# david-strejc/fei

Measured on AMD Instinct MI355X. Metric: agent tok/s (llama3-8b local decode, 1 agent/GPU), higher is better.
Workload: dtype bf16; 1 GPU; model=llama3-8b, global_batch=1, seq_len=512, parallelism=dp1 (1 agent per GPU, weak scaling), hip_graph=True, stream_engine=False

## Files before the change

fei_amd/models/llama.py:

```python

from __future__ import annotations

import math
import os
from dataclasses import dataclass
from typing import Dict, List, Optional

import torch
import torch.nn.functional as F

from fei_amd import ops
from fei_amd.engine.config import ModelSpec
from fei_amd.ops import reference as ref
from fei_amd.parallel.pg import ParallelContext, all_gather_cat, all_reduce_sum


@dataclass
class LayerWeights:
    norm_attn: torch.Tensor
    wqkv: torch.Tensor
    wo: torch.Tensor
    norm_mlp: torch.Tensor
    wgu: torch.Tensor
    wdown: torch.Tensor
# ... 7 lines not shown
        dtype: torch.dtype = torch.bfloat16,
        tp: Optional[ParallelContext] = None,
        seed: int = 1234,
        max_seq_len: Optional[int] = None,
    ):
        self.spec = spec
        self.device = device
        self.dtype = dtype
        self.tp = tp or ParallelContext()
        self.max_seq_len = max_seq_len or spec.max_seq_len
        tp_size = self.tp.world_size if self.tp.is_distributed else 1
        if spec.num_kv_heads % tp_size or spec.num_heads % tp_size or \
                spec.intermediate_size % tp_size or spec.vocab_size % tp_size:
            raise ValueError(f"model {spec.name} not divisible by tp={tp_size}")
        self.tp_size = tp_size
        self.tp_rank = self.tp.rank if self.tp.is_distributed else 0
        self.hq_l = spec.num_heads // tp_size
        self.hkv_l = spec.num_kv_heads // tp_size
        self.inter_l = spec.intermediate_size // tp_size
        self.vocab_l = spec.vocab_size // tp_size
        self.D = spec.head_dim
        self._init_weights(seed)
        self.rope = ref.rope_table(self.max_seq_len, self.D, spec.rope_theta,
                                   device=device)
        self.prefetch_mb = int(os.environ.get("FEI_PREFETCH", "0") or 0)
        self._pf_stream = None
        self._pf_sink = None
        self.norm_precomp = os.environ.get("FEI_NORM_PRECOMP", "0") == "1"


    def _rand(self, gen, *shape, scale: float) -> torch.Tensor:
        w = torch.randn(*shape, generator=gen, device=self.device,
                        dtype=torch.float32) * scale
        return w.to(self.dtype)

    def _init_weights(self, seed: int) -> None:
        s = self.spec
        gen = torch.Generator(device=self.device)
        gen.manual_seed(seed)
        C = s.hidden_size
        sc = 1.0 / math.sqrt(C)
        self.emb = self._rand(gen, s.vocab_size, C, scale=0.02)
        self.layers: List[LayerWeights] = []
        r = self.tp_rank
        for _ in range(s.num_layers):
            wq = self._rand(gen, s.num_heads * self.D, C, scale=sc)
            wk = self._rand(gen, s.num_kv_heads * self.D, C, scale=sc)
            wv = self._rand(gen, s.num_kv_heads * self.D, C, scale=sc)
            wo = self._rand(gen, C, s.num_heads * self.D, scale=sc / math.sqrt(2 * s.num_layers))
            wg = self._rand(gen, s.intermediate_size, C, scale=sc)
            wu = self._rand(gen, s.intermediate_size, C, scale=sc)
            wd = self._rand(gen, C, s.intermediate_size,
                            scale=1.0 / math.sqrt(s.intermediate_size) / math.sqrt(2 * s.num_layers))
            wq = wq.view(s.num_heads, self.D, C)[r * self.hq_l:(r + 1) * self.hq_l].reshape(-1, C)
            wk = wk.view(s.num_kv_heads, self.D, C)[r * self.hkv_l:(r + 1) * self.hkv_l].reshape(-1, C)
            wv = wv.view(s.num_kv_heads, self.D, C)[r * self.hkv_l:(r + 1) * self.hkv_l].reshape(-1, C)
            wo = wo.view(C, s.num_heads, self.D)[:, r * self.hq_l:(r + 1) * self.hq_l].reshape(C, -1)
            wg = wg[r * self.inter_l:(r + 1) * self.inter_l]
            wu = wu[r * self.inter_l:(r + 1) * self.inter_l]
            wd = wd[:, r * self.inter_l:(r + 1) * self.inter_l]
            self.layers.append(LayerWeights(
                norm_attn=torch.ones(C, device=self.device, dtype=self.dtype),
                wqkv=torch.cat([wq, wk, wv], dim=0).contiguous(),
                wo=wo.contiguous(),
                norm_mlp=torch.ones(C, device=self.device, dtype=self.dtype),
                wgu=torch.cat([wg, wu], dim=0).contiguous(),
                wdown=wd.contiguous(),
            ))
        self.norm_f = torch.ones(C, device=self.device, dtype=self.dtype)
        lm = self._rand(gen, s.vocab_size, C, scale=sc)
        self.lm_head = lm[r * self.vocab_l:(r + 1) * self.vocab_l].contiguous()
        self.vocab_offset = r * self.vocab_l

    def quantize_fp8(self) -> None:
        self.fp8 = []
        for lw in self.layers:
            self.fp8.append({
                "wqkv": ops.quant_fp8(lw.wqkv),
                "wo": ops.quant_fp8(lw.wo),
                "wgu": ops.quant_fp8(lw.wgu),
                "wdown": ops.quant_fp8(lw.wdown),
            })
        self.fp8_lm_head = ops.quant_fp8(self.lm_head)

    def param_bytes(self) -> int:
        total = self.emb.numel() + self.norm_f.numel() + self.lm_head.numel()
        for lw in self.layers:
            for t in (lw.norm_attn, lw.wqkv, lw.wo, lw.norm_mlp, lw.wgu, lw.wdown):
                total += t.numel()
        return total * self.emb.element_size()


    def new_kv_cache(self, batch: int, max_seq: Optional[int] = None,
                     kv_quant: Optional[str] = None):
        max_seq = max_seq or self.max_seq_len
        shape = (batch, self.hkv_l, max_seq, self.D)
        if kv_quant == "fp8":
            return (
                [ops.QuantKV.zeros(shape, self.device)
                 for _ in range(self.spec.num_layers)],
                [ops.QuantKV.zeros(shape, self.device)
                 for _ in range(self.spec.num_layers)],
            )
        if kv_quant is not None:
            raise ValueError(f"unknown kv_quant {kv_quant!r}")
        return (
            [torch.zeros(shape, device=self.device, dtype=self.dtype)
             for _ in range(self.spec.num_layers)],
            [torch.zeros(shape, device=self.device, dtype=self.dtype)
             for _ in range(self.spec.num_layers)],
        )


    def _qkv_views(self, qkv: torch.Tensor, B: int, S: Optional[int] = None):
        D = self.D
        W = qkv.shape[-1]
        off_k = self.hq_l * D
        off_v = off_k + self.hkv_l * D
        if S is None:
            q = qkv.as_strided((B, self.hq_l, D), (W, D, 1))
            k = qkv.as_strided((B, self.hkv_l, D), (W, D, 1), storage_offset=qkv.storage_offset() + off_k)
            v = qkv.as_strided((B, self.hkv_l, D), (W, D, 1), storage_offset=qkv.storage_offset() + off_v)
        else:
            q = qkv.as_strided((B, S, self.hq_l, D), (S * W, W, D, 1))
            k = qkv.as_strided((B, S, self.hkv_l, D), (S * W, W, D, 1), storage_offset=qkv.storage_offset() + off_k)
            v = qkv.as_strided((B, S, self.hkv_l, D), (S * W, W, D, 1), storage_offset=qkv.storage_offset() + off_v)
        return q, k, v


    def forward_decode(
        self,
        token: torch.Tensor,
        pos: torch.Tensor,
        k_caches: List[torch.Tensor],
        v_caches: List[torch.Tensor],
        attn_splits: int = 32,
        workspace=None,
        fused_attn: bool = False,
        attn_out: Optional[torch.Tensor] = None,
        fused_norm: bool = False,
        gather_logits: bool = True,
    ) -> torch.Tensor:
        if fused_norm and self.tp_size == 1 and token.shape[0] == 1 and \
                self.spec.hidden_size * 2 <= 32 * 1024:
            return self._forward_decode_fused_norm(
                token, pos, k_caches, v_caches, attn_splits, workspace,
                fused_attn, attn_out)
        s = self.spec
        B = token.shape[0]
        h = F.embedding(token.long(), self.emb)
        scale = 1.0 / math.sqrt(self.D)
        n_layers = len(self.layers)
        x = ops.rmsnorm(h, self.layers[0].norm_attn, s.norm_eps)
        for li, lw in enumerate(self.layers):
            qkv = ops.linear_decode(x, lw.wqkv)
            q, k, v = self._qkv_views(qkv, B)
            if fused_attn:
                att = ops.attn_decode_fused(q, k, v, k_caches[li],
                                            v_caches[li], pos, self.rope,
                                            scale=scale, out=attn_out)
            else:
                att = ops.attn_decode(q, k_caches[li], v_caches[li], pos,
                                      splits=attn_splits, scale=scale,
                                      workspace=workspace, out=attn_out,
                                      k=k, v=v, table=self.rope, layer=li)
            o = ops.linear_decode(att.reshape(B, -1), lw.wo)
            all_reduce_sum(o, self.tp)
            x, h = ops.fused_add_rmsnorm(o, h, lw.norm_mlp, s.norm_eps)
            act = ops.gemv_swiglu(x, lw.wgu)
            d = ops.linear_decode(act, lw.wdown)
            all_reduce_sum(d, self.tp)
            next_norm = (self.layers[li + 1].norm_attn if li + 1 < n_layers
                         else self.norm_f)
            x, h = ops.fused_add_rmsnorm(d, h, next_norm, s.norm_eps)
        logits = ops.linear_decode(x, self.lm_head)
        if gather_logits:
            logits = all_gather_cat(logits, dim=-1, ctx=self.tp)
        return logits

    def forward_decode_stream(self, token, pos, k_caches, v_caches,
                              ws: dict, bufs) -> torch.Tensor:
        s = self.spec
        h = F.embedding(token.long(), self.emb)
        bufs[0].copy_(h.to(bufs[0].dtype))
        scale = 1.0 / math.sqrt(self.D)
        cur, nxt = bufs
        for li, lw in enumerate(self.layers):
            ops.stream_layer(cur, nxt, lw, s, k_caches[li], v_caches[li],
                             self.rope, pos, ws, li, scale)
            cur, nxt = nxt, cur
        return ops.gemv_norm(cur, self.norm_f, self.lm_head, s.norm_eps)

    def _ssq_slots(self, B: int, device) -> torch.Tensor:
        buf = getattr(self, "_ssq", None)
        if buf is None or buf.shape[1] != B or buf.device != device:
            buf = torch.zeros(2 * len(self.layers), B, dtype=torch.float32,
                              device=device)
            self._ssq = buf
        return buf

    def _forward_decode_fused_norm(self, token, pos, k_caches, v_caches,
                                   attn_splits, workspace, fused_attn,
                                   attn_out):
        s = self.spec
        B = token.shape[0]
        fp8 = getattr(self, "fp8", None)
        if fp8 is not None and (B != 1 or s.hidden_size * 2 > 32 * 1024):
            fp8 = None
        h = F.embedding(token.long(), self.emb).contiguous()
        scale = 1.0 / math.sqrt(self.D)
        ssq = (self._ssq_slots(B, h.device)
               if (self.norm_precomp and fp8 is None and h.is_cuda) else None)
        if ssq is not None:
            ssq.zero_()
        pf = self.prefetch_mb > 0 and fp8 is None and h.is_cuda
        if pf and self._pf_stream is None:
            self._pf_stream = torch.cuda.Stream()
            self._pf_sink = torch.zeros(1, dtype=torch.float32,
                                        device=h.device)
        for li, lw in enumerate(self.layers):
            if fp8 is not None:
                q8 = fp8[li]
                qkv = ops.gemv_norm_fp8(h, lw.norm_attn, *q8["wqkv"],
                                        s.norm_eps)
            else:
                qkv = ops.gemv_norm(
                    h, lw.norm_attn, lw.wqkv, s.norm_eps,
                    ssq=ssq[2 * li - 1] if (ssq is not None and li > 0) else None)
            if pf:
                ev = torch.cuda.Event()
                ev.record()
                with torch.cuda.stream(self._pf_stream):
                    self._pf_stream.wait_event(ev)
                    ops.prefetch(lw.wgu, self.prefetch_mb << 20,
                                 self._pf_sink)
            q, k, v = self._qkv_views(qkv, B)
            if fused_attn:
                att = ops.attn_decode_fused(q, k, v, k_caches[li],
                                            v_caches[li], pos, self.rope,
                                            scale=scale, out=attn_out)
            else:
                att = ops.attn_decode(q, k_caches[li], v_caches[li], pos,
                                      splits=attn_splits, scale=scale,
                                      workspace=workspace, out=attn_out,
                                      k=k, v=v, table=self.rope, layer=li)
            if fp8 is not None:
                ops.gemv_res_fp8(att.reshape(B, -1), *q8["wo"], h)
                act = ops.gemv_swiglu_norm_fp8(h, lw.norm_mlp, *q8["wgu"],
                                               s.norm_eps)
                ops.gemv_res_fp8(act, *q8["wdown"], h)
            else:
                ops.gemv_res(att.reshape(B, -1), lw.wo, h,
                             ssq_out=ssq[2 * li] if ssq is not None else None)
                act = ops.gemv_swiglu_norm(
                    h, lw.norm_mlp, lw.wgu, s.norm_eps,
                    ssq=ssq[2 * li] if ssq is not None else None)
                ops.gemv_res(act, lw.wdown, h,
                             ssq_out=ssq[2 * li + 1] if ssq is not None else None)
        if pf:
            torch.cuda.current_stream().wait_stream(self._pf_stream)
        if fp8 is not None:
            return ops.gemv_norm_fp8(h, self.norm_f, *self.fp8_lm_head,
                                     s.norm_eps)
        return ops.gemv_norm(h, self.norm_f, self.lm_head, s.norm_eps,
                             ssq=ssq[-1] if ssq is not None else None)

    def forward_prefill(
        self,
        tokens: torch.Tensor,
        pos0: torch.Tensor,
        k_caches: List[torch.Tensor],
        v_caches: List[torch.Tensor],
        all_positions: bool = False,
    ) -> torch.Tensor:
        s = self.spec
        B, S = tokens.shape
        h = F.embedding(tokens.long(), self.emb)
        scale = 1.0 / math.sqrt(self.D)
        n_layers = len(self.layers)
        x = ops.rmsnorm(h, self.layers[0].norm_attn, s.norm_eps)
        for li, lw in enumerate(self.layers):
            qkv = F.linear(x, lw.wqkv)
            qkv2 = qkv.view(B * S, -1)
            q, k, v = self._qkv_views(qkv2, B, S)
            ops.rope_kv_prefill(q, k, v, k_caches[li], v_caches[li], pos0, self.rope)
            att = ops.attn_prefill(q, k_caches[li], v_caches[li], pos0, scale=scale)
            o = F.linear(att.reshape(B, S, -1), lw.wo)
            all_reduce_sum(o, self.tp)
            x, h = ops.fused_add_rmsnorm(o, h, lw.norm_mlp, s.norm_eps)
            gu = F.linear(x, lw.wgu)
            act = ops.swiglu(gu)
            d = F.linear(act, lw.wdown)
            all_reduce_sum(d, self.tp)
            next_norm = (self.layers[li + 1].norm_attn if li + 1 < n_layers
                         else self.norm_f)
            x, h = ops.fused_add_rmsnorm(d, h, next_norm, s.norm_eps)
        last = x if all_positions else x[:, -1, :]
        logits = F.linear(last, self.lm_head)
        logits = all_gather_cat(logits, dim=-1, ctx=self.tp)
        return logits


    def state_dict_full(self) -> Dict[str, torch.Tensor]:
        if self.tp_size != 1:
            raise RuntimeError("state_dict_full requires tp=1 (save from an "
                               "unsharded model; any-tp models can LOAD it)")
        s = self.spec
        out: Dict[str, torch.Tensor] = {
            "emb": self.emb, "norm_f": self.norm_f, "lm_head": self.lm_head,
        }
        for i, lw in enumerate(self.layers):
            qd = s.num_heads * self.D
            kvd = s.num_kv_heads * self.D
            out[f"layers.{i}.wq"] = lw.wqkv[:qd]
            out[f"layers.{i}.wk"] = lw.wqkv[qd:qd + kvd]
            out[f"layers.{i}.wv"] = lw.wqkv[qd + kvd:]
            out[f"layers.{i}.wo"] = lw.wo
            out[f"layers.{i}.wg"] = lw.wgu[:s.intermediate_size]
            out[f"layers.{i}.wu"] = lw.wgu[s.intermediate_size:]
            out[f"layers.{i}.wd"] = lw.wdown
            out[f"layers.{i}.norm_attn"] = lw.norm_attn
            out[f"layers.{i}.norm_mlp"] = lw.norm_mlp
        return out

# ... 46 lines not shown
```

fei_amd/ops/__init__.py:

```python

from __future__ import annotations

import ctypes
import math
import os
from typing import Optional, Tuple

import torch

from fei_amd.ops import reference as ref

_LIB: Optional[ctypes.CDLL] = None
_LIB_ERR: Optional[str] = None
_LIB_PATH = os.path.join(os.path.dirname(os.path.abspath(__file__)),
                         "libfei_kernels.so")

_c = ctypes
_vp, _i, _f, _u64, _l = _c.c_void_p, _c.c_int, _c.c_float, _c.c_ulonglong, _c.c_long


def _try_load() -> None:
    global _LIB, _LIB_ERR
    if _LIB is not None or _LIB_ERR is not None:
        return
    try:
        lib = ctypes.CDLL(_LIB_PATH)
    except OSError as e:
        _LIB_ERR = str(e)
        return
    lib.fei_rmsnorm.argtypes = [_vp, _vp, _vp, _i, _i, _f, _vp]
    lib.fei_add_rmsnorm.argtypes = [_vp, _vp, _vp, _vp, _i, _i, _f, _vp]
    lib.fei_rope_kv_decode.argtypes = [_vp, _vp, _vp, _vp, _vp, _vp, _vp,
                                       _i, _i, _i, _i, _i, _l, _l, _vp]
    lib.fei_rope_kv_prefill.argtypes = [_vp, _vp, _vp, _vp, _vp, _vp, _vp,
                                        _i, _i, _i, _i, _i, _i, _l, _l, _vp]
    lib.fei_attn_decode.argtypes = [_vp, _vp, _vp, _vp, _vp, _vp,
                                    _i, _i, _i, _i, _i, _i, _f, _l,
                                    _vp, _vp, _vp, _l, _vp, _vp, _i, _vp]
    lib.fei_attn_decode_combine.argtypes = [_vp, _vp, _vp, _i, _i, _i, _i, _vp]
    lib.fei_swiglu.argtypes = [_vp, _vp, _l, _i, _vp]
    lib.fei_sample.argtypes = [_vp, _vp, _vp, _vp, _vp, _i, _i, _i, _f, _u64,
                               _i, _vp]
    lib.fei_advance.argtypes = [_vp, _vp, _i, _i, _vp]
    lib.fei_attn_prefill.argtypes = [_vp, _vp, _vp, _vp, _vp, _vp,
                                     _i, _i, _i, _i, _i, _i, _f, _i, _l, _vp]
    lib.fei_mfma_probe.argtypes = [_vp, _vp, _vp, _vp]
    lib.fei_gemv.argtypes = [_vp, _vp, _vp, _i, _i, _i, _i, _vp]
    lib.fei_gemm_m8.argtypes = [_vp, _vp, _vp, _i, _i, _i, _i, _vp]
    lib.fei_attn_decode_fused.argtypes = [_vp, _vp, _vp, _vp, _vp, _vp, _vp,
                                          _vp, _i, _i, _i, _i, _i, _f,
                                          _l, _l, _vp]
    lib.fei_sample_onepass.argtypes = [_vp, _vp, _vp, _vp, _i, _i, _f, _u64,
                                       _i, _vp]
    lib.fei_sample_shard.argtypes = [_vp, _vp, _vp, _i, _i, _i, _f, _u64, _vp]
    lib.fei_sample_filtered.argtypes = [_vp, _vp, _vp, _vp, _vp, _i, _i, _i,
                                        _f, _f, _u64, _i, _vp]
    lib.fei_rope_kv8_decode.argtypes = [_vp, _vp, _vp, _vp, _vp, _vp, _vp,
                                        _vp, _vp, _i, _i, _i, _i, _i, _l, _l,
                                        _vp]
    lib.fei_rope_kv8_prefill.argtypes = [_vp, _vp, _vp, _vp, _vp, _vp, _vp,
                                         _vp, _vp, _i, _i, _i, _i, _i, _i,
                                         _l, _l, _vp]
    lib.fei_attn_decode_kv8.argtypes = [_vp, _vp, _vp, _vp, _vp, _vp, _vp,
                                        _vp, _i, _i, _i, _i, _i, _i, _f, _l,
                                        _vp, _vp, _vp, _l, _vp]
    lib.fei_attn_decode_kv8.restype = _i
    lib.fei_attn_prefill_kv8.argtypes = [_vp, _vp, _vp, _vp, _vp, _vp, _vp,
                                         _i, _i, _i, _i, _i, _i, _f, _l, _vp]
    lib.fei_attn_prefill_kv8.restype = _i
    lib.fei_stream_layer_check.argtypes = [_i, _i, _i, _i, _i]
    lib.fei_stream_layer_check.restype = _i
    lib.fei_stream_layer.argtypes = [_vp, _vp, _vp, _vp, _vp, _vp, _vp, _vp,
                                     _vp, _vp, _vp, _vp, _vp, _vp, _vp, _vp,
                                     _vp, _vp, _vp, _i, _i, _i, _i, _i,
                                     _i, _i, _f, _f, _vp]
    lib.fei_attn_decode_paged.argtypes = [_vp, _vp, _vp, _vp, _vp, _vp, _vp,
                                          _i, _i, _i, _i, _i, _i, _i, _f,
                                          _l, _vp, _vp, _vp, _l, _vp]
    lib.fei_add_layernorm.argtypes = [_vp, _vp, _vp, _vp, _vp, _i, _i, _f,
                                      _i, _vp]
    lib.fei_gelu.argtypes = [_vp, _vp, _l, _vp]
    lib.fei_gemv_norm_fp8.argtypes = [_vp, _vp, _vp, _vp, _vp, _i, _i, _i,
                                      _f, _vp]
    lib.fei_gemv_res_fp8.argtypes = [_vp, _vp, _vp, _vp, _i, _i, _i, _vp]
    lib.fei_gemv_swiglu_norm_fp8.argtypes = [_vp, _vp, _vp, _vp, _vp, _i, _i,
                                             _i, _f, _vp]
    lib.fei_quant_fp8_rows.argtypes = [_vp, _vp, _vp, _i, _i, _vp]
    lib.fei_gemv_swiglu.argtypes = [_vp, _vp, _vp, _i, _i, _i, _i, _vp]
    lib.fei_prefetch.argtypes = [_vp, _l, _vp, _i, _vp]
    lib.fei_gemv_res.argtypes = [_vp, _vp, _vp, _i, _i, _i, _i, _vp, _vp]
    lib.fei_gemv_norm.argtypes = [_vp, _vp, _vp, _vp, _i, _i, _i, _f, _i, _vp,
                                  _vp]
    lib.fei_gemv_swiglu_norm.argtypes = [_vp, _vp, _vp, _vp, _i, _i, _i, _f,
                                         _i, _vp, _vp]
    _LIB = lib


def kernels_available() -> bool:
    _try_load()
    return _LIB is not None


def require_lib() -> ctypes.CDLL:
    _try_load()
    if _LIB is None:
        raise RuntimeError(
            "fei_amd HIP kernel library not found at "
            f"{_LIB_PATH} ({_LIB_ERR}). Build it with "
            "`python -m fei_amd.ops.build` — GPU execution refuses to fall "
            "back to eager PyTorch.")
    return _LIB


def _stream() -> int:
    return torch.cuda.current_stream().cuda_stream


def _ptr(t: torch.Tensor) -> int:
    return t.data_ptr()




class QuantKV:

    __slots__ = ("data", "scale")

    def __init__(self, data: torch.Tensor, scale: torch.Tensor):
        assert data.dtype == torch.uint8 and scale.dtype == torch.float32
        assert tuple(scale.shape) == tuple(data.shape[:-1])
        assert data.is_contiguous() and scale.is_contiguous(), \
            "QuantKV needs contiguous data and scale"
        assert data.data_ptr() % 16 == 0, "QuantKV data must be 16 B aligned"
        self.data = data
        self.scale = scale

    @classmethod
    def zeros(cls, shape, device) -> "QuantKV":
        return cls(torch.zeros(shape, dtype=torch.uint8, device=device),
                   torch.ones(shape[:-1], dtype=torch.float32, device=device))

    @property
    def shape(self):
        return self.data.shape

    def dequant(self, length: Optional[int] = None) -> torch.Tensor:
        n = self.data.shape[2] if length is None else length
        return ref.dequant_kv_fp8(self.data[:, :, :n], self.scale[:, :, :n])


def _kv8_pair(k_cache, v_cache) -> bool:
    k8, v8 = isinstance(k_cache, QuantKV), isinstance(v_cache, QuantKV)
    if k8 != v8:
        raise TypeError("k_cache and v_cache must both be QuantKV or both "
                        "be tensors")
    return k8


def _check_gqa(name: str, Hq: int, Hkv: int) -> None:
    if Hkv <= 0 or Hq % Hkv != 0 or Hq // Hkv not in (1, 2, 4, 8):
        raise ValueError(f"{name}: unsupported GQA group Hq={Hq}, Hkv={Hkv} "
                         "(Hq/Hkv must be 1, 2, 4 or 8)")


def _check_vec8(name: str, n: int, what: str = "last dimension") -> None:
    if n % 8 != 0:
        raise ValueError(f"{name}: {what} must be a multiple of 8, got {n}")


def rmsnorm(x: torch.Tensor, weight: torch.Tensor, eps: float = 1e-5,
            out: Optional[torch.Tensor] = None) -> torch.Tensor:
    _check_vec8("rmsnorm", x.shape[-1])
    if x.numel() == 0:
        return torch.empty_like(x) if out is None else out
    if not x.is_cuda:
        return ref.rmsnorm(x, weight, eps)
    lib = require_lib()
    x2 = x.contiguous()
    if out is None:
        out = torch.empty_like(x2)
    rows = x2.numel() // x2.shape[-1]
    lib.fei_rmsnorm(_ptr(out), _ptr(x2), _ptr(weight), rows, x2.shape[-1],
                    eps, _stream())
    return out


def fused_add_rmsnorm(x: torch.Tensor, residual: torch.Tensor,
                      weight: torch.Tensor, eps: float = 1e-5,
                      out: Optional[torch.Tensor] = None
                      ) -> Tuple[torch.Tensor, torch.Tensor]:
    _check_vec8("fused_add_rmsnorm", x.shape[-1])
    if not residual.is_contiguous():
        raise ValueError("fused_add_rmsnorm: residual must be contiguous "
                         "(it is updated in place)")
    if x.numel() == 0:
        return (torch.empty_like(x) if out is None else out), residual
    if not x.is_cuda:
        o, res = ref.fused_add_rmsnorm(x, residual, weight, eps)
        residual.copy_(res)
        return o, residual
    lib = require_lib()
    x2 = x.contiguous()
    if out is None:
        out = torch.empty_like(x2)
    rows = x2.numel() // x2.shape[-1]
    lib.fei_add_rmsnorm(_ptr(out), _ptr(residual), _ptr(x2), _ptr(weight),
                        rows, x2.shape[-1], eps, _stream())
    return out, residual


def rope_kv_decode(q, k, v, k_cache, v_cache, pos, table) -> torch.Tensor:
    kv8 = _kv8_pair(k_cache, v_cache)
    if not q.is_cuda:
        if kv8:
            q_out = ref.rope_kv_decode_fp8(
                q, k, v, k_cache.data, k_cache.scale, v_cache.data,
                v_cache.scale, pos, table)
        else:
            q_out = ref.rope_kv_decode(q, k, v, k_cache, v_cache, pos, table)
        q.copy_(q_out)
        return q
    lib = require_lib()
    B, Hq, D = q.shape
    Hkv = k.shape[1]
    assert q.stride(2) == 1 and q.stride(1) == D, "head rows must be contiguous"
    assert k.stride(1) == D and v.stride(1) == D
    assert k.stride(0) == v.stride(0)
    if kv8:
        assert D in (64, 128), f"fp8 KV append supports D in (64,128), got {D}"
        lib.fei_rope_kv8_decode(_ptr(q), _ptr(k), _ptr(v), _ptr(k_cache.data),
                                _ptr(k_cache.scale), _ptr(v_cache.data),
                                _ptr(v_cache.scale), _ptr(table), _ptr(pos),
                                B, Hq, Hkv, D, k_cache.shape[2],
                                q.stride(0), k.stride(0), _stream())
        return q
    lib.fei_rope_kv_decode(_ptr(q), _ptr(k), _ptr(v), _ptr(k_cache),
                           _ptr(v_cache), _ptr(table), _ptr(pos),
                           B, Hq, Hkv, D, k_cache.shape[2],
                           q.stride(0), k.stride(0), _stream())
    return q


def rope_kv_prefill(q, k, v, k_cache, v_cache, pos0, table) -> torch.Tensor:
    kv8 = _kv8_pair(k_cache, v_cache)
    if not q.is_cuda:
        if kv8:
            q_out = ref.rope_kv_prefill_fp8(
# ... 241 lines not shown
    rows = gu.numel() // gu.shape[-1]
    if out is None:
        out = torch.empty(*gu.shape[:-1], inter, dtype=gu.dtype, device=gu.device)
    lib.fei_swiglu(_ptr(out), _ptr(gu), rows, inter, _stream())
    return out


def sample(logits: torch.Tensor, token: torch.Tensor,
           step: torch.Tensor, workspace: torch.Tensor,
           out_tokens: Optional[torch.Tensor] = None,
           temperature: float = 0.0, seed: int = 0,
           nchunks: int = 64) -> torch.Tensor:
    B, V = logits.shape
    if not logits.is_cuda:
        if temperature <= 0:
            t = ref.argmax_sample(logits)
        else:
            g = torch.Generator().manual_seed(
                (int(seed) * 1000003 + int(step)) & 0x7FFFFFFF)
            t = ref.gumbel_sample(logits, temperature, g)
        token.copy_(t)
        if out_tokens is not None:
            st = int(step)
            for b in range(B):
                if st < out_tokens.shape[1]:
                    out_tokens[b, st] = t[b]
        return token
    lib = require_lib()
    max_new = out_tokens.shape[1] if out_tokens is not None else 0
    out_ptr = _ptr(out_tokens) if out_tokens is not None else None
    if B <= 8:
        lib.fei_sample_onepass(_ptr(logits), _ptr(token), out_ptr, _ptr(step),
                               B, V, temperature, seed, max_new, _stream())
    else:
        lib.fei_sample(_ptr(logits), _ptr(token), out_ptr, _ptr(step),
                       _ptr(workspace), B, V, nchunks, temperature, seed,
                       max_new, _stream())
    return token


def sample_filtered(logits: torch.Tensor, token: torch.Tensor,
                    step: torch.Tensor, info: torch.Tensor,
                    out_tokens: Optional[torch.Tensor] = None,
                    temperature: float = 0.0, seed: int = 0,
                    top_k: int = 0, top_p: float = 1.0) -> torch.Tensor:
    if top_k < 0:
        raise ValueError(f"top_k must be >= 0, got {top_k}")
    if not 0.0 < top_p <= 1.0:
        raise ValueError(f"top_p must be in (0, 1], got {top_p}")
    B, V = logits.shape
    if not logits.is_cuda:
        keep, thr, count = ref.filter_keep(logits, top_k, top_p)
        info[:, 0] = thr
        info[:, 1].view(torch.int32).copy_(count)
        if keep.all():
            masked = logits
        else:
            masked = logits.float().masked_fill(~keep, float("-inf"))
        return sample(masked, token, step, None, out_tokens=out_tokens,
                      temperature=temperature, seed=seed)
    lib = require_lib()
    max_new = out_tokens.shape[1] if out_tokens is not None else 0
    out_ptr = _ptr(out_tokens) if out_tokens is not None else None
    lib.fei_sample_filtered(_ptr(logits), _ptr(token), out_ptr, _ptr(step),
                            _ptr(info), B, V, int(top_k), float(top_p),
                            float(temperature), int(seed), max_new, _stream())
    return token


def sample_shard(logits: torch.Tensor, step: torch.Tensor,
                 v_offset: int, out: torch.Tensor,
                 temperature: float = 0.0, seed: int = 0) -> torch.Tensor:
    B, Vl = logits.shape
    if not logits.is_cuda:
        vals = logits.float()
        if temperature > 0:
            vals = vals / temperature + ref.hash_gumbel(
                B, Vl, v_offset, int(seed), int(step))
        best = vals.max(dim=-1)
        out[:, 0] = best.values
        out[:, 1].view(torch.int32).copy_(
            (best.indices + v_offset).to(torch.int32))
        return out
    lib = require_lib()
    lib.fei_sample_shard(_ptr(logits), _ptr(out), _ptr(step), B, Vl,
                         int(v_offset), float(temperature), int(seed),
                         _stream())
    return out



STREAM_NSPLIT = 32


def stream_layer_check(C: int, Hq: int, Hkv: int, D: int, I: int) -> int:
    lib = require_lib()
    return int(lib.fei_stream_layer_check(C, Hq, Hkv, D, I))


def stream_workspace(spec, device) -> dict:
    C, D = spec.hidden_size, spec.head_dim
    Hq, Hkv, I = spec.num_heads, spec.num_kv_heads, spec.intermediate_size
    mk = lambda n: torch.zeros(n, dtype=torch.int64, device=device)
    return {
        "g_qkv": mk((Hq + 2 * Hkv) * D),
        "g_att": mk(Hq * D // 2),
        "g_h2": mk(C // 2),
        "g_act": mk(I),
        "g_done": mk(6 * 256),
        "fail": torch.zeros(1, dtype=torch.int32, device=device),
    }


def stream_layer(x_in: torch.Tensor, h_out: torch.Tensor, lw, spec,
                 k_cache: torch.Tensor, v_cache: torch.Tensor,
                 cos_sin: torch.Tensor, pos: torch.Tensor, ws: dict,
                 layer: int, scale: float) -> None:
    lib = require_lib()
    lib.fei_stream_layer(
        _ptr(x_in), _ptr(h_out), _ptr(lw.wqkv), _ptr(lw.wo), _ptr(lw.wgu),
        _ptr(lw.wdown), _ptr(lw.norm_attn), _ptr(lw.norm_mlp),
        _ptr(k_cache), _ptr(v_cache), _ptr(cos_sin), _ptr(pos),
        _ptr(ws["g_qkv"]), _ptr(ws["g_att"]),
        _ptr(ws["g_h2"]), _ptr(ws["g_act"]), _ptr(ws["g_done"]),
        _ptr(ws["dbg"]) if "dbg" in ws else None,
        _ptr(ws["fail"]),
        spec.hidden_size, spec.num_heads, spec.num_kv_heads, spec.head_dim,
        spec.intermediate_size, k_cache.shape[-2], layer, spec.norm_eps,
        scale, _stream())


def advance(pos: torch.Tensor, step: torch.Tensor,
            max_pos: int = 1 << 30) -> None:
    if not pos.is_cuda:
        pos.clamp_(max=max_pos - 1)
        pos += 1
        step += 1
        return
    lib = require_lib()
    lib.fei_advance(_ptr(pos), _ptr(step), pos.shape[0], max_pos, _stream())


def mfma_probe(A: torch.Tensor, B: torch.Tensor) -> torch.Tensor:
    lib = require_lib()
    C = torch.empty(16, 16, dtype=torch.float32, device=A.device)
    lib.fei_mfma_probe(_ptr(A.contiguous()), _ptr(B.contiguous()), _ptr(C),
                       _stream())
    return C



_GEMV_NT_MIN_BYTES = int(os.environ.get("FEI_GEMV_NT_MIN", 0))
_FUSED_CMB = os.environ.get("FEI_FUSED_CMB", "0") == "1"


def _gemm_m8_ok(M: int, N: int, K: int) -> bool:
    return 4 <= M <= 8 and K % 1024 == 0 and N % 16 == 0


def _gemv_ok(M: int, K: int) -> bool:
    return M in (1, 2, 4, 8) and K % 8 == 0


def linear_decode(x: torch.Tensor, w: torch.Tensor,
                  out: Optional[torch.Tensor] = None) -> torch.Tensor:
    M = x.numel() // x.shape[-1]
    K = x.shape[-1]
    N = w.shape[0]
    if not x.is_cuda or not (_gemv_ok(M, K) or _gemm_m8_ok(M, N, K)):
        return torch.nn.functional.linear(x, w)
    lib = require_lib()
    x2 = x.contiguous().view(M, K)
    if out is None:
        out = torch.empty(*x.shape[:-1], N, dtype=x.dtype, device=x.device)
    nt = 1 if (N * K * 2 >= _GEMV_NT_MIN_BYTES) else 0
    if _gemm_m8_ok(M, N, K):
        lib.fei_gemm_m8(_ptr(out), _ptr(x2), _ptr(w), M, N, K, 0,
                        _stream())
        return out
    lib.fei_gemv(_ptr(out), _ptr(x2), _ptr(w), M, N, K, nt, _stream())
    return out


def gemv_swiglu(x: torch.Tensor, wgu: torch.Tensor,
                out: Optional[torch.Tensor] = None) -> torch.Tensor:
    M = x.numel() // x.shape[-1]
    K = x.shape[-1]
    I = wgu.shape[0] // 2
    if not x.is_cuda:
        return ref.swiglu(torch.nn.functional.linear(x, wgu))
    if not (_gemv_ok(M, K) or _gemm_m8_ok(M, 2 * I, K)):
        return swiglu(torch.nn.functional.linear(x, wgu))
    lib = require_lib()
    x2 = x.contiguous().view(M, K)
    if out is None:
        out = torch.empty(*x.shape[:-1], I, dtype=x.dtype, device=x.device)
    nt = 1 if (2 * I * K * 2 >= _GEMV_NT_MIN_BYTES) else 0
    if _gemm_m8_ok(M, 2 * I, K):
        gu = torch.empty(M, 2 * I, dtype=x.dtype, device=x.device)
        lib.fei_gemm_m8(_ptr(gu), _ptr(x2), _ptr(wgu), M, 2 * I, K, 0,
                        _stream())
        lib.fei_swiglu(_ptr(out), _ptr(gu), M, I, _stream())
        return out
    lib.fei_gemv_swiglu(_ptr(out), _ptr(x2), _ptr(wgu), M, I, K, nt,
                        _stream())
    return out


def gemv_res(x: torch.Tensor, w: torch.Tensor, res: torch.Tensor,
             ssq_out: Optional[torch.Tensor] = None) -> torch.Tensor:
    M = x.numel() // x.shape[-1]
    K = x.shape[-1]
    N = w.shape[0]
    if not x.is_cuda or not _gemv_ok(M, K):
        lin = torch.nn.functional.linear(x, w)
        res.copy_((res.float() + lin.float().view_as(res)).to(res.dtype))
        return res
    lib = require_lib()
    x2 = x.contiguous().view(M, K)
    nt = 1 if (N * K * 2 >= _GEMV_NT_MIN_BYTES) else 0
    lib.fei_gemv_res(_ptr(res), _ptr(x2), _ptr(w), M, N, K, nt,
                     _ptr(ssq_out) if ssq_out is not None else None,
                     _stream())
    return res


def gemv_norm(res: torch.Tensor, wnorm: torch.Tensor, w: torch.Tensor,
              eps: float = 1e-5,
              out: Optional[torch.Tensor] = None,
              ssq: Optional[torch.Tensor] = None) -> torch.Tensor:
    M = res.numel() // res.shape[-1]
    K = res.shape[-1]
    N = w.shape[0]
    if not res.is_cuda or not _gemv_ok(M, K):
        return torch.nn.functional.linear(rmsnorm(res, wnorm, eps), w)
    lib = require_lib()
    r2 = res.contiguous().view(M, K)
    if out is None:
        out = torch.empty(*res.shape[:-1], N, dtype=res.dtype, device=res.device)
    nt = 1 if (N * K * 2 >= _GEMV_NT_MIN_BYTES) else 0
    lib.fei_gemv_norm(_ptr(out), _ptr(r2), _ptr(wnorm), _ptr(w), M, N, K,
                      eps, nt, _ptr(ssq) if ssq is not None else None,
                      _stream())
    return out


def gemv_swiglu_norm(res: torch.Tensor, wnorm: torch.Tensor,
                     wgu: torch.Tensor, eps: float = 1e-5,
                     out: Optional[torch.Tensor] = None,
                     ssq: Optional[torch.Tensor] = None) -> torch.Tensor:
    M = res.numel() // res.shape[-1]
    K = res.shape[-1]
    I = wgu.shape[0] // 2
    if not res.is_cuda or not _gemv_ok(M, K):
        gu = torch.nn.functional.linear(rmsnorm(res, wnorm, eps).float(),
                                        wgu.float())
        return ref.swiglu(gu).to(res.dtype)
    lib = require_lib()
    r2 = res.contiguous().view(M, K)
    if out is None:
        out = torch.empty(*res.shape[:-1], I, dtype=res.dtype, device=res.device)
    nt = 1 if (wgu.shape[0] * K * 2 >= _GEMV_NT_MIN_BYTES) else 0
    lib.fei_gemv_swiglu_norm(_ptr(out), _ptr(r2), _ptr(wnorm), _ptr(wgu),
                             M, I, K, eps, nt,
                             _ptr(ssq) if ssq is not None else None,
                             _stream())
    return out


def prefetch(w: torch.Tensor, max_bytes: int, sink: torch.Tensor,
             n_blocks: int = 512, stream=None) -> None:
    if not w.is_cuda:
        return
    lib = require_lib()
    bytes_ = min(max_bytes, w.numel() * w.element_size())
    sp = stream if stream is not None else _stream()
    lib.fei_prefetch(_ptr(w), bytes_, _ptr(sink), n_blocks, sp)


def attn_decode_paged(q, k_pool, v_pool, block_table, pos, splits: int = 32,
                      scale: Optional[float] = None,
                      workspace: Optional[Tuple[torch.Tensor, torch.Tensor]] = None,
                      out: Optional[torch.Tensor] = None,
                      k: Optional[torch.Tensor] = None,
                      v: Optional[torch.Tensor] = None,
                      table: Optional[torch.Tensor] = None) -> torch.Tensor:
    B, Hq, D = q.shape
    n_blocks, Hkv, BS, _ = k_pool.shape
    assert BS & (BS - 1) == 0, "block size must be a power of two"
    bs_log = BS.bit_length() - 1
    scale = scale if scale is not None else 1.0 / math.sqrt(D)
    if not q.is_cuda:
        if table is not None:
            q = ref.apply_rope(q, pos.long(), table).to(q.dtype)
            k_r = ref.apply_rope(k, pos.long(), table).to(k.dtype)
            for b in range(B):
                p = int(pos[b])
                blk = int(block_table[b, p >> bs_log])
                k_pool[blk, :, p & (BS - 1), :] = k_r[b]
                v_pool[blk, :, p & (BS - 1), :] = v[b]
        max_len = block_table.shape[1] * BS
        kc = torch.zeros(B, Hkv, max_len, D, dtype=k_pool.dtype)
        vc = torch.zeros_like(kc)
        for b in range(B):
            for j, blk in enumerate(block_table[b].tolist()):
                if blk < 0:
                    continue
                kc[b, :, j * BS:(j + 1) * BS] = k_pool[blk]
                vc[b, :, j * BS:(j + 1) * BS] = v_pool[blk]
        return ref.attn_decode(q, kc, vc, pos + 1, scale)
    lib = require_lib()
    _check_gqa("attn_decode_paged", Hq, Hkv)
    if workspace is None:
        part_o = torch.empty(B, Hq, splits, D, dtype=torch.float32, device=q.device)
        part_ml = torch.empty(B, Hq, splits, 2, dtype=torch.float32, device=q.device)
    else:
        part_o, part_ml = workspace
        assert part_o.shape[2] == splits and part_ml.shape[2] == splits
    if out is None:
        out = torch.empty_like(q)
    assert q.stride(2) == 1 and q.stride(1) == D
    assert D in (64, 128), f"paged attention supports D in (64,128), got {D}"
    assert splits <= 64
    if table is not None:
        assert k is not None and v is not None
        assert k.stride(1) == D and k.stride(0) == v.stride(0)
        kin, vin, cs, kv_bs = _ptr(k), _ptr(v), _ptr(table), k.stride(0)
    else:
        kin = vin = cs = None
        kv_bs = 0
    lib.fei_attn_decode_paged(_ptr(q), _ptr(k_pool), _ptr(v_pool),
                              _ptr(block_table), _ptr(part_o), _ptr(part_ml),
                              _ptr(pos), B, Hq, Hkv, D, bs_log,
                              block_table.shape[1], splits, scale,
                              q.stride(0), kin, vin, cs, kv_bs, _stream())
    lib.fei_attn_decode_combine(_ptr(out), _ptr(part_o), _ptr(part_ml),
                                B, Hq, D, splits, _stream())
    return out


def layernorm(x: torch.Tensor, weight: torch.Tensor, bias: torch.Tensor,
              eps: float = 1e-5, residual: Optional[torch.Tensor] = None,
              out: Optional[torch.Tensor] = None) -> torch.Tensor:
    _check_vec8("layernorm", x.shape[-1])
    if x.numel() == 0:
        return torch.empty_like(x) if out is None else out
    if not x.is_cuda:
        return ref.layernorm(x, weight, bias, eps, residual)
    lib = require_lib()
    x2 = x.contiguous()
    rows = x2.numel() // x2.shape[-1]
    if out is None:
        out = torch.empty_like(x2)
    res_ptr = _ptr(residual.contiguous()) if residual is not None else _ptr(x2)
    lib.fei_add_layernorm(_ptr(out), _ptr(x2), res_ptr, _ptr(weight),
                          _ptr(bias), rows, x2.shape[-1], eps,
                          1 if residual is not None else 0, _stream())
    return out


def gelu(x: torch.Tensor, out: Optional[torch.Tensor] = None) -> torch.Tensor:
    _check_vec8("gelu", x.numel(), "element count")
    if x.numel() == 0:
        return torch.empty_like(x) if out is None else out
    if not x.is_cuda:
        return ref.gelu(x)
    lib = require_lib()
    x2 = x.contiguous()
    if out is None:
        out = torch.empty_like(x2)
    lib.fei_gelu(_ptr(out), _ptr(x2), x2.numel(), _stream())
    return out



def quant_fp8(w: torch.Tensor):
    if not w.is_cuda:
        return ref.quant_fp8(w)
    lib = require_lib()
    N, K = w.shape
    w8 = torch.empty(N, K, dtype=torch.uint8, device=w.device)
    scales = torch.empty(N, dtype=torch.float32, device=w.device)
    lib.fei_quant_fp8_rows(_ptr(w8), _ptr(scales), _ptr(w.contiguous()),
                           N, K, _stream())
    return w8, scales


def _gemv_fp8_ok(M: int, K: int) -> bool:
    return M in (1, 2, 4, 8) and K % 16 == 0


def _linear_fp8(x: torch.Tensor, w8: torch.Tensor,
                wscale: torch.Tensor) -> torch.Tensor:
    codes = w8.view(torch.float8_e4m3fn).float()
    return torch.nn.functional.linear(x.float(), codes) * wscale.float()


def gemv_norm_fp8(res, wnorm, w8, wscale, eps: float = 1e-5,
                  out: Optional[torch.Tensor] = None) -> torch.Tensor:
    M = res.numel() // res.shape[-1]
    K = res.shape[-1]
    N = w8.shape[0]
    if not res.is_cuda or not _gemv_fp8_ok(M, K):
        return _linear_fp8(rmsnorm(res, wnorm, eps), w8, wscale).to(res.dtype)
    assert M * K * 2 <= 64 * 1024, \
        "fp8 norm-GEMV stages M*K bf16 activations in LDS (<=64 KB)"
    lib = require_lib()
    r2 = res.contiguous().view(M, K)
    if out is None:
        out = torch.empty(*res.shape[:-1], N, dtype=res.dtype, device=res.device)
    lib.fei_gemv_norm_fp8(_ptr(out), _ptr(r2), _ptr(wnorm), _ptr(w8),
                          _ptr(wscale), M, N, K, eps, _stream())
    return out


def gemv_res_fp8(x, w8, wscale, res) -> torch.Tensor:
    M = x.numel() // x.shape[-1]
    K = x.shape[-1]
    N = w8.shape[0]
# ... 28 lines not shown
```

fei_amd/ops/build.py:

```python

from __future__ import annotations

import os
import subprocess
import sys

CSRC = os.path.join(os.path.dirname(os.path.abspath(__file__)), "csrc")
OUT = os.path.join(os.path.dirname(os.path.abspath(__file__)), "libfei_kernels.so")
SOURCES = ["fei_kernels.hip", "attn_prefill.hip", "gemv.hip", "attn_decode_fused.hip", "gemv_fp8.hip", "stream_layer.hip",
           "sample_filtered.hip", "kv_fp8.hip"]
HIPCC = os.environ.get("HIPCC", "hipcc")
ARCH = os.environ.get("FEI_AMD_ARCH", "gfx950")


def needs_build() -> bool:
    if not os.path.exists(OUT):
        return True
    out_mtime = os.path.getmtime(OUT)
    for src in SOURCES + ["fei_common.h"]:
        if os.path.getmtime(os.path.join(CSRC, src)) > out_mtime:
            return True
    return False


def build(force: bool = False, verbose: bool = True) -> str:
    if not force and not needs_build():
        return OUT
    cmd = [
        HIPCC, f"--offload-arch={ARCH}", "-O3", "-std=c++17",
        "-shared", "-fPIC",
        *[os.path.join(CSRC, s) for s in SOURCES],
        "-o", OUT,
    ]
    if verbose:
        print("[fei_amd.ops.build]", " ".join(cmd), file=sys.stderr)
    result = subprocess.run(cmd, capture_output=True, text=True)
    if result.returncode != 0:
        raise RuntimeError(
            f"hipcc failed (rc={result.returncode}):\n{result.stderr[-4000:]}")
    return OUT


if __name__ == "__main__":
    build(force="--force" in sys.argv)
    print(OUT)
```

Before: 296.1 tok/s.

## Fuse residual add and RMSNorm into the prologue of QKV and gate-up GEMVs

Adds new HIP kernels that compute residual add plus RMSNorm redundantly in every block, then run the bf16 GEMV (and the SwiGLU GEMV) against the normalized vector held in LDS. Weight-row preloads are issued before the norm so the norm latency overlaps with the weight fetch. The decode loop now uses ping-pong residual buffers, and block 0 writes the new residual. This removes two separate add+norm launches per layer and their global round trips, at the cost of every block redoing the norm and reading delta, residual and norm weight.

```diff
diff --git a/fei_amd/models/llama.py b/fei_amd/models/llama.py
--- a/fei_amd/models/llama.py
+++ b/fei_amd/models/llama.py
@@ -183,8 +183,22 @@
         scale = 1.0 / math.sqrt(self.D)
         n_layers = len(self.layers)
         x = ops.rmsnorm(h, self.layers[0].norm_attn, s.norm_eps)
+        addnorm = (ops._ADDNORM_GEMV and self.tp_size == 1 and B == 1
+                   and h.is_cuda and h.dtype == torch.bfloat16
+                   and ops._addnorm_ok(B, s.hidden_size))
+        if addnorm:
+            h = h.contiguous()
+            hb = torch.empty(2, B, s.hidden_size, dtype=h.dtype,
+                             device=h.device)
+            nbuf = 0
+        d = None
         for li, lw in enumerate(self.layers):
-            qkv = ops.linear_decode(x, lw.wqkv)
+            if addnorm and li > 0:
+                qkv = ops.gemv_addnorm(d, h, hb[nbuf], lw.norm_attn, lw.wqkv,
+                                       s.norm_eps)
+                h, nbuf = hb[nbuf], nbuf ^ 1
+            else:
+                qkv = ops.linear_decode(x, lw.wqkv)
             q, k, v = self._qkv_views(qkv, B)
             if fused_attn:
                 att = ops.attn_decode_fused(q, k, v, k_caches[li],
@@ -197,10 +211,17 @@
                                       k=k, v=v, table=self.rope, layer=li)
             o = ops.linear_decode(att.reshape(B, -1), lw.wo)
             all_reduce_sum(o, self.tp)
-            x, h = ops.fused_add_rmsnorm(o, h, lw.norm_mlp, s.norm_eps)
-            act = ops.gemv_swiglu(x, lw.wgu)
+            if addnorm:
+                act = ops.gemv_swiglu_addnorm(o, h, hb[nbuf], lw.norm_mlp,
+                                              lw.wgu, s.norm_eps)
+                h, nbuf = hb[nbuf], nbuf ^ 1
+            else:
+                x, h = ops.fused_add_rmsnorm(o, h, lw.norm_mlp, s.norm_eps)
+                act = ops.gemv_swiglu(x, lw.wgu)
             d = ops.linear_decode(act, lw.wdown)
             all_reduce_sum(d, self.tp)
+            if addnorm and li + 1 < n_layers:
+                continue
             next_norm = (self.layers[li + 1].norm_attn if li + 1 < n_layers
                          else self.norm_f)
             x, h = ops.fused_add_rmsnorm(d, h, next_norm, s.norm_eps)
diff --git a/fei_amd/ops/__init__.py b/fei_amd/ops/__init__.py
--- a/fei_amd/ops/__init__.py
+++ b/fei_amd/ops/__init__.py
@@ -93,6 +93,10 @@
                                   _vp]
     lib.fei_gemv_swiglu_norm.argtypes = [_vp, _vp, _vp, _vp, _i, _i, _i, _f,
                                          _i, _vp, _vp]
+    for fn in (lib.fei_gemv_addnorm, lib.fei_gemv_swiglu_addnorm):
+        fn.argtypes = [_vp, _vp, _vp, _vp, _vp, _vp, _i, _i, _i, _f, _i, _i,
+                       _vp]
+        fn.restype = _i
     _LIB = lib
 
 
@@ -640,6 +644,7 @@
 
 _GEMV_NT_MIN_BYTES = int(os.environ.get("FEI_GEMV_NT_MIN", 0))
 _FUSED_CMB = os.environ.get("FEI_FUSED_CMB", "0") == "1"
+_ADDNORM_GEMV = os.environ.get("FEI_ADDNORM_GEMV", "1") == "1"
 
 
 def _gemm_m8_ok(M: int, N: int, K: int) -> bool:
@@ -753,6 +758,85 @@
                              M, I, K, eps, nt,
                              _ptr(ssq) if ssq is not None else None,
                              _stream())
+    return out
+
+
+
+_ADDNORM_ROW_GROUPS = max(1, int(os.environ.get("FEI_ADDNORM_RG", "2") or 2))
+_ADDNORM_ROW_GROUPS_SWIGLU = max(
+    1, int(os.environ.get("FEI_ADDNORM_RG_SWIGLU", "2") or 2))
+
+
+def _addnorm_ok(M: int, K: int) -> bool:
+    return M == 1 and _gemv_ok(M, K) and M * K * 2 <= 32 * 1024
+
+
+def _addnorm_check(name: str, delta, res_in, res_out) -> None:
+    if not res_in.is_contiguous() or not res_out.is_contiguous():
+        raise ValueError(f"{name}: res_in and res_out must be contiguous")
+    if res_in.shape != res_out.shape or res_in.dtype != res_out.dtype:
+        raise ValueError(f"{name}: res_in and res_out must match in shape "
+                         "and dtype")
+    if delta.shape != res_in.shape:
+        raise ValueError(f"{name}: delta must have the residual's shape")
+    a0, b0 = res_in.data_ptr(), res_out.data_ptr()
+    nbytes = res_in.numel() * res_in.element_size()
+    if a0 < b0 + nbytes and b0 < a0 + nbytes:
+        raise ValueError(f"{name}: res_in and res_out must not share storage "
+                         "(the new residual cannot be written in place)")
+
+
+def gemv_addnorm(delta: torch.Tensor, res_in: torch.Tensor,
+                 res_out: torch.Tensor, wnorm: torch.Tensor, w: torch.Tensor,
+                 eps: float = 1e-5,
+                 out: Optional[torch.Tensor] = None) -> torch.Tensor:
+    _addnorm_check("gemv_addnorm", delta, res_in, res_out)
+    K = res_in.shape[-1]
+    M = res_in.numel() // max(K, 1)
+    N = w.shape[0]
+    if not res_in.is_cuda or not _addnorm_ok(M, K):
+        res_out.copy_(res_in)
+        x, _ = fused_add_rmsnorm(delta, res_out, wnorm, eps)
+        return linear_decode(x, w, out=out)
+    lib = require_lib()
+    d2 = delta.contiguous()
+    if out is None:
+        out = torch.empty(*res_in.shape[:-1], N, dtype=res_in.dtype,
+                          device=res_in.device)
+    nt = 1 if (N * K * 2 >= _GEMV_NT_MIN_BYTES) else 0
+    rc = lib.fei_gemv_addnorm(_ptr(out), _ptr(d2), _ptr(res_in),
+                              _ptr(res_out), _ptr(wnorm), _ptr(w), M, N, K,
+                              eps, nt, _ADDNORM_ROW_GROUPS, _stream())
+    if rc != 0:
+        raise RuntimeError(f"fei_gemv_addnorm refused the launch (rc={rc})")
+    return out
+
+
+def gemv_swiglu_addnorm(delta: torch.Tensor, res_in: torch.Tensor,
+                        res_out: torch.Tensor, wnorm: torch.Tensor,
+                        wgu: torch.Tensor, eps: float = 1e-5,
+                        out: Optional[torch.Tensor] = None) -> torch.Tensor:
+    _addnorm_check("gemv_swiglu_addnorm", delta, res_in, res_out)
+    K = res_in.shape[-1]
+    M = res_in.numel() // max(K, 1)
+    I = wgu.shape[0] // 2
+    if not res_in.is_cuda or not _addnorm_ok(M, K):
+        res_out.copy_(res_in)
+        x, _ = fused_add_rmsnorm(delta, res_out, wnorm, eps)
+        return gemv_swiglu(x, wgu, out=out)
+    lib = require_lib()
+    d2 = delta.contiguous()
+    if out is None:
+        out = torch.empty(*res_in.shape[:-1], I, dtype=res_in.dtype,
+                          device=res_in.device)
+    nt = 1 if (wgu.shape[0] * K * 2 >= _GEMV_NT_MIN_BYTES) else 0
+    rc = lib.fei_gemv_swiglu_addnorm(_ptr(out), _ptr(d2), _ptr(res_in),
+                                     _ptr(res_out), _ptr(wnorm), _ptr(wgu),
+                                     M, I, K, eps, nt,
+                                     _ADDNORM_ROW_GROUPS_SWIGLU, _stream())
+    if rc != 0:
+        raise RuntimeError(
+            f"fei_gemv_swiglu_addnorm refused the launch (rc={rc})")
     return out
 
 
diff --git a/fei_amd/ops/build.py b/fei_amd/ops/build.py
--- a/fei_amd/ops/build.py
+++ b/fei_amd/ops/build.py
@@ -8,7 +8,7 @@
 CSRC = os.path.join(os.path.dirname(os.path.abspath(__file__)), "csrc")
 OUT = os.path.join(os.path.dirname(os.path.abspath(__file__)), "libfei_kernels.so")
 SOURCES = ["fei_kernels.hip", "attn_prefill.hip", "gemv.hip", "attn_decode_fused.hip", "gemv_fp8.hip", "stream_layer.hip",
-           "sample_filtered.hip", "kv_fp8.hip"]
+           "sample_filtered.hip", "kv_fp8.hip", "gemv_addnorm.hip"]
 HIPCC = os.environ.get("HIPCC", "hipcc")
 ARCH = os.environ.get("FEI_AMD_ARCH", "gfx950")
 
diff --git a/fei_amd/ops/csrc/gemv_addnorm.hip b/fei_amd/ops/csrc/gemv_addnorm.hip
--- /dev/null
+++ b/fei_amd/ops/csrc/gemv_addnorm.hip
@@ -0,0 +1,267 @@
+#include "fei_common.h"
+
+namespace {
+
+constexpr int PRE = 8;
+constexpr int PRO = 2;
+
+template <bool NT>
+__device__ __forceinline__ s16x8 ldw(const s16x8* p) {
+  return NT ? __builtin_nontemporal_load(p) : *p;
+}
+
+template <bool NT>
+__device__ __forceinline__ void preload_row(s16x8 (&wv)[PRE],
+                                            const s16x8* __restrict__ wrow,
+                                            int nv, int lane) {
+#pragma unroll
+  for (int u = 0; u < PRE; ++u)
+    wv[u] = ldw<NT>(&wrow[min(lane + u * 64, nv - 1)]);
+}
+
+struct AddnormIn { s16x8 d[PRO], h[PRO], w[PRO]; };
+
+__device__ __forceinline__ void addnorm_issue(AddnormIn& in,
+                                              const s16x8* __restrict__ dr,
+                                              const s16x8* __restrict__ hr,
+                                              const s16x8* __restrict__ wr,
+                                              int nv, int tid) {
+#pragma unroll
+  for (int u = 0; u < PRO; ++u) {
+    const int i = min(tid + u * 256, nv - 1);
+    in.d[u] = dr[i];
+    in.h[u] = hr[i];
+    in.w[u] = wr[i];
+  }
+}
+
+__device__ __forceinline__ float addnorm_sumsq8(s16x8 rv, s16x8 xv, s16x8& nr,
+                                                float ss) {
+#pragma unroll
+  for (int j = 0; j < 8; ++j) {
+    float f = bf2f((u16)rv[j]) + bf2f((u16)xv[j]);
+    u16 b = f2bf(f);
+    nr[j] = (short)b;
+    f = bf2f(b);
+    ss = fmaf(f, f, ss);
+  }
+  return ss;
+}
+
+__device__ __forceinline__ s16x8 addnorm_scale8(s16x8 rv, s16x8 wvv,
+                                                float inv) {
+  s16x8 o;
+#pragma unroll
+  for (int j = 0; j < 8; ++j)
+    o[j] = (short)f2bf(bf2f((u16)rv[j]) * inv * bf2f((u16)wvv[j]));
+  return o;
+}
+
+__device__ __forceinline__ void addnorm_finish(const AddnormIn& in,
+                                               s16x8* xs, float* red,
+                                               const s16x8* __restrict__ dr,
+                                               const s16x8* __restrict__ hr,
+                                               const s16x8* __restrict__ wr,
+                                               s16x8* __restrict__ ho,
+                                               int nv, int K, float eps,
+                                               int tid) {
+  float ss = 0.f;
+  s16x8 nr[PRO];
+#pragma unroll
+  for (int u = 0; u < PRO; ++u) {
+    const int i = tid + u * 256;
+    const float s2 = addnorm_sumsq8(in.h[u], in.d[u], nr[u], ss);
+    ss = i < nv ? s2 : ss;
+    if (ho && i < nv) ho[i] = nr[u];
+  }
+  for (int i = tid + PRO * 256; i < nv; i += 256) {
+    s16x8 n;
+    ss = addnorm_sumsq8(hr[i], dr[i], n, ss);
+    xs[i] = n;
+    if (ho) ho[i] = n;
+  }
+  ss = block_reduce_sum(ss, red);
+  const float inv = rsqrtf(ss / (float)K + eps);
+#pragma unroll
+  for (int u = 0; u < PRO; ++u) {
+    const int i = tid + u * 256;
+    const s16x8 o = addnorm_scale8(nr[u], in.w[u], inv);
+    if (i < nv) xs[i] = o;
+  }
+  for (int i = tid + PRO * 256; i < nv; i += 256)
+    xs[i] = addnorm_scale8(xs[i], wr[i], inv);
+  __syncthreads();
+}
+
+template <bool NT>
+__device__ __forceinline__ void dot_rows(float& acc0, float& acc1,
+                                         const s16x8 (&wv0)[PRE],
+                                         const s16x8 (&wv1)[PRE],
+                                         const s16x8* __restrict__ wrow0,
+                                         const s16x8* __restrict__ wrow1,
+                                         const s16x8* xs, int nv, int lane) {
+#pragma unroll
+  for (int u = 0; u < PRE; ++u) {
+    const int i = lane + u * 64;
+    const s16x8 xv = xs[min(i, nv - 1)];
+    const float d0 = dot8_bf16(xv, wv0[u]);
+    const float d1 = dot8_bf16(xv, wv1[u]);
+    acc0 = i < nv ? acc0 + d0 : acc0;
+    acc1 = i < nv ? acc1 + d1 : acc1;
+    __builtin_amdgcn_sched_barrier(0);
+  }
+  for (int i = lane + PRE * 64; i < nv; i += 64) {
+    const s16x8 a = ldw<NT>(&wrow0[i]);
+    const s16x8 b = ldw<NT>(&wrow1[i]);
+    const s16x8 xv = xs[i];
+    acc0 += dot8_bf16(xv, a);
+    acc1 += dot8_bf16(xv, b);
+  }
+}
+
+#define ADDNORM_LDS(K) ((size_t)(K) * 2 + 4 * sizeof(float))
+
+template <int M, bool NT>
+__global__ void __launch_bounds__(256)
+k_gemv_addnorm(u16* __restrict__ out, const u16* __restrict__ delta,
+               const u16* __restrict__ h_in, u16* __restrict__ h_out,
+               const u16* __restrict__ wn, const u16* __restrict__ w,
+               int N, int K, float eps, int rg) {
+  static_assert(M == 1, "the add+norm prologue is batch-1 only");
+  extern __shared__ s16x8 lds_x[];
+  s16x8* xs = lds_x;
+  float* red = (float*)(lds_x + (K >> 3));
+  const int tid = threadIdx.x;
+  const int lane = tid & 63;
+  const int wid = tid >> 6;
+  const int nv = K >> 3;
+  int n0 = blockIdx.x * rg * 8 + wid * 2;
+
+  bool active = n0 < N;
+  bool two = (n0 + 1) < N;
+  const s16x8* wrow0 = (const s16x8*)(w + (long)(active ? n0 : 0) * K);
+  const s16x8* wrow1 =
+      (const s16x8*)(w + (long)(active ? n0 + (two ? 1 : 0) : 0) * K);
+
+  const s16x8* dr = (const s16x8*)delta;
+  const s16x8* hr = (const s16x8*)h_in;
+  const s16x8* wr = (const s16x8*)wn;
+  AddnormIn in;
+  addnorm_issue(in, dr, hr, wr, nv, tid);
+  s16x8 wv0[PRE], wv1[PRE];
+  preload_row<NT>(wv0, wrow0, nv, lane);
+  preload_row<NT>(wv1, wrow1, nv, lane);
+  addnorm_finish(in, xs, red, dr, hr, wr,
+                 blockIdx.x == 0 ? (s16x8*)h_out : nullptr, nv, K, eps, tid);
+
+  for (int g = 0;;) {
+    float acc0 = 0.f, acc1 = 0.f;
+    dot_rows<NT>(acc0, acc1, wv0, wv1, wrow0, wrow1, xs, nv, lane);
+    const float v0 = wave_reduce_sum(acc0);
+    const float v1 = wave_reduce_sum(acc1);
+    if (lane == 0 && active) {
+      out[n0] = f2bf(v0);
+      if (two) out[n0 + 1] = f2bf(v1);
+    }
+    if (++g >= rg) break;
+    n0 += 8;
+    active = n0 < N;
+    two = (n0 + 1) < N;
+    wrow0 = (const s16x8*)(w + (long)(active ? n0 : 0) * K);
+    wrow1 = (const s16x8*)(w + (long)(active ? n0 + (two ? 1 : 0) : 0) * K);
+    preload_row<NT>(wv0, wrow0, nv, lane);
+    preload_row<NT>(wv1, wrow1, nv, lane);
+  }
+}
+
+template <int M, bool NT>
+__global__ void __launch_bounds__(256)
+k_gemv_swiglu_addnorm(u16* __restrict__ out, const u16* __restrict__ delta,
+                      const u16* __restrict__ h_in, u16* __restrict__ h_out,
+                      const u16* __restrict__ wn, const u16* __restrict__ w,
+                      int N, int K, float eps, int rg) {
+  static_assert(M == 1, "the add+norm prologue is batch-1 only");
+  extern __shared__ s16x8 lds_x[];
+  s16x8* xs = lds_x;
+  float* red = (float*)(lds_x + (K >> 3));
+  const int tid = threadIdx.x;
+  const int lane = tid & 63;
+  const int wid = tid >> 6;
+  const int nv = K >> 3;
+  int n = blockIdx.x * rg * 4 + wid;
+
+  bool active = n < N;
+  const s16x8* grow = (const s16x8*)(w + (long)(active ? n : 0) * K);
+  const s16x8* urow = (const s16x8*)(w + (long)((active ? n : 0) + N) * K);
+
+  const s16x8* dr = (const s16x8*)delta;
+  const s16x8* hr = (const s16x8*)h_in;
+  const s16x8* wr = (const s16x8*)wn;
+  AddnormIn in;
+  addnorm_issue(in, dr, hr, wr, nv, tid);
+  s16x8 gv[PRE], uv[PRE];
+  preload_row<NT>(gv, grow, nv, lane);
+  preload_row<NT>(uv, urow, nv, lane);
+  addnorm_finish(in, xs, red, dr, hr, wr,
+                 blockIdx.x == 0 ? (s16x8*)h_out : nullptr, nv, K, eps, tid);
+
+  for (int g = 0;;) {
+    float accg = 0.f, accu = 0.f;
+    dot_rows<NT>(accg, accu, gv, uv, grow, urow, xs, nv, lane);
+    const float gs = wave_reduce_sum(accg);
+    const float us = wave_reduce_sum(accu);
+    if (lane == 0 && active) {
+      const float silu = gs / (1.f + __expf(-gs));
+      out[n] = f2bf(silu * us);
+    }
+    if (++g >= rg) break;
+    n += 4;
+    active = n < N;
+    grow = (const s16x8*)(w + (long)(active ? n : 0) * K);
+    urow = (const s16x8*)(w + (long)((active ? n : 0) + N) * K);
+    preload_row<NT>(gv, grow, nv, lane);
+    preload_row<NT>(uv, urow, nv, lane);
+  }
+}
+
+}
+
+extern "C" {
+
+int fei_gemv_addnorm(void* out, const void* delta, const void* h_in,
+                     void* h_out, const void* wn, const void* w, int M, int N,
+                     int K, float eps, int nontemporal, int row_groups,
+                     hipStream_t stream) {
+  if (M != 1) return -1;
+  if (K <= 0 || K % 8 != 0 || (size_t)K * 2 > 32 * 1024 || N < 1) return -2;
+  if (h_in == h_out) return -3;
+  const int rg = row_groups < 1 ? 1 : row_groups;
+  const int groups = (N + 7) / 8;
+  dim3 grid((groups + rg - 1) / rg);
+#define LA(NTV) hipLaunchKernelGGL((k_gemv_addnorm<1, NTV>), grid, dim3(256), \
+    ADDNORM_LDS(K), stream, (u16*)out, (const u16*)delta, (const u16*)h_in, \
+    (u16*)h_out, (const u16*)wn, (const u16*)w, N, K, eps, rg)
+  if (nontemporal) LA(true); else LA(false);
+#undef LA
+  return 0;
+}
+
+int fei_gemv_swiglu_addnorm(void* out, const void* delta, const void* h_in,
+                            void* h_out, const void* wn, const void* w, int M,
+                            int N, int K, float eps, int nontemporal,
+                            int row_groups, hipStream_t stream) {
+  if (M != 1) return -1;
+  if (K <= 0 || K % 8 != 0 || (size_t)K * 2 > 32 * 1024 || N < 1) return -2;
+  if (h_in == h_out) return -3;
+  const int rg = row_groups < 1 ? 1 : row_groups;
+  const int groups = (N + 3) / 4;
+  dim3 grid((groups + rg - 1) / rg);
+#define LA(NTV) hipLaunchKernelGGL((k_gemv_swiglu_addnorm<1, NTV>), grid, \
+    dim3(256), ADDNORM_LDS(K), stream, (u16*)out, (const u16*)delta, \
+    (const u16*)h_in, (u16*)h_out, (const u16*)wn, (const u16*)w, N, K, eps, rg)
+  if (nontemporal) LA(true); else LA(false);
+#undef LA
+  return 0;
+}
+
+}
```

New measurement: 311.7 tok/s (median of 6 runs). +5.3%, better.
